# rkhosrowshahi/MO-VAE

Hardware: NVIDIA B200
Metric: aggregation_GBps (higher is better)
Workload: dtype f32

## Files before the change

mo-vae_b200/csrc/aggregate.cu:

```cuda
#include "recombine_device.cuh"
#include "solve_device.cuh"

namespace movae {

int fill_solve_params(int k, const movae_solve_spec* spec, SolveParams* out);
int check_solve_vectors(const SolveParams& p, const float* d_vec, const float* d_aux);

constexpr int kAggThreads = 256;
static_assert(kAggThreads == kGramThreads && kAggThreads == kRecThreads && kAggThreads == kSolveThreads, "one CTA shape");

struct AggArgs {
    const float* J;
    int64_t P, ldJ;
    unsigned char* ws;
    const float* vec;
    const float* aux;
    float* out;
    int accumulate;
    float* w_out;
    double* diag_out;
    double* G_out;
    int64_t window_gram;
    int64_t window_rec;
};

constexpr double kL2WindowFraction = 0.55;

struct PolicyIO {
    uint64_t pol;
    __device__ __forceinline__ float4 load(const float4* p) const { return ld_stream_f4(p, pol); }
    __device__ __forceinline__ float load(const float* p) const { return ld_stream_f1(p, pol); }
};

template <bool LAST_USE>
struct WindowSteps {
    int64_t window;
    __device__ __forceinline__ PolicyIO operator()(int64_t d) const {
        return {(d < window) == LAST_USE ? l2_policy_evict_first() : l2_policy_evict_normal()};
    }
};

template <int K>
__device__ __forceinline__ void aggregate_solve_phase(const SolveParams& sp, const P2PArgs& px, const float* vec, const float* aux,
                                                      float* w_out, double* diag_out, double* G_out, const GramWorkspace& ws,
                                                      unsigned int ready0, unsigned long long t_start) {
    __shared__ SolveSmem S;
    __shared__ double Gs[K * K];
    __shared__ unsigned long long seq_s;
    __shared__ int failed_s;
    const int tid = threadIdx.x;
    const unsigned long long t_in = global_timer_ns();
    gram_combine_partials<K>(ws.partials, Gs);
    if (tid == 0) { *ws.ticket = 0u; failed_s = 0; ws.stamps[4] = global_timer_ns(); }
    if (px.world > 0) {
        XchgBuffer* own = px.peers[px.rank];
        if (tid == 0) seq_s = own->step + 1;
        __syncthreads();
        const unsigned long long seq = seq_s;
        const int par = (int)(seq & 1ull);
        if (tid < K * K) {
            const double v = Gs[tid];
            for (int r = 0; r < px.world; ++r) st_relaxed_sys_f64(&px.peers[r]->slots[par][px.rank][tid], v);
        }
        __threadfence_system();
        __syncthreads();
        if (tid < px.world) st_release_sys_u64(&px.peers[tid]->flags[par][px.rank], seq);
        if (tid == 0) own->step = seq;
        if (tid < px.world && !wait_flag_sys(&own->flags[par][tid], seq, kExchangeTimeoutNs)) failed_s = 1;
        __syncthreads();
        if (tid < K * K) {
            double g = 0.0;
            for (int r = 0; r < px.world; ++r) g += ld_relaxed_sys_f64(&own->slots[par][r][tid]);
            Gs[tid] = g;
        }
        __syncthreads();
    }
    if (tid == 0) ws.stamps[5] = global_timer_ns();
    if (tid < MK * MK) {
        const int i = tid / MK, j = tid % MK;
        S.G[i][j] = (i < K && j < K) ? Gs[i * K + j] : 0.0;
    }
    if (G_out && tid < K * K) G_out[tid] = Gs[tid];
    __syncthreads();
    solve_block<K>(sp, S, vec, aux, failed_s != 0, tid);
    if (tid < K) {
        w_out[tid] = S.w[tid];
        if (sp.comfort) w_out[K + tid] = S.w2[tid];
    }
    __syncthreads();
    if (tid == 0) {
        ws.stamps[0] = t_start;
        ws.stamps[1] = t_in;
        ws.stamps[2] = global_timer_ns();
        __threadfence();
        st_release_gpu_u32(ws.ready, ready0 + 1u);
    }
    solve_diagnostics(sp, S, tid);
    __syncthreads();
    if (tid < MOVAE_DIAG_DOUBLES && diag_out) diag_out[tid] = S.dg[tid];
}

__device__ __forceinline__ void aggregate_prologue(const GramWorkspace& ws, unsigned int& ready0, unsigned long long& t_start) {
    if (threadIdx.x == 0) {
        ready0 = ld_acquire_gpu_u32(ws.ready);
        t_start = global_timer_ns();
    }
}

__device__ __forceinline__ void aggregate_wait_ready(const unsigned int* ready, unsigned int ready0) {
    if (threadIdx.x == 0) {
        const unsigned long long t0 = global_timer_ns();
        while (ld_acquire_gpu_u32(ready) == ready0) {
            __nanosleep(40);
            if (global_timer_ns() - t0 > 2ull * kExchangeTimeoutNs) break;
        }
    }
    __syncthreads();
}

__device__ __forceinline__ void aggregate_epilogue(const GramWorkspace& ws) {
    __syncthreads();
    if (threadIdx.x == 0) {
        if (atomicAdd(ws.exit, 1u) == gridDim.x - 1) {
            ws.stamps[3] = global_timer_ns();
            *ws.exit = 0u;
        }
    }
}

template <int K, int U1, int U2, bool VEC, int MINB>
__global__ void __launch_bounds__(kAggThreads, MINB)
aggregate_kernel(AggArgs a, SolveParams sp, P2PArgs px) {
    constexpr int NACC = GramAcc<K>::N;
    const GramWorkspace ws(a.ws);
    __shared__ unsigned int ready0;
    __shared__ unsigned long long t_start;
    __shared__ double red[kGramThreads / 32][NACC];
    __shared__ int is_last;
    aggregate_prologue(ws, ready0, t_start);

    double acc64[NACC];
#pragma unroll
    for (int i = 0; i < NACC; ++i) acc64[i] = 0.0;
    gram_stream_tiles<K, U1, VEC>(a.J, a.P, a.ldJ, acc64, WindowSteps<false>{a.window_gram});
    const bool last = gram_cta_partial_and_ticket<K>(acc64, ws.partials, ws.ticket, red, &is_last);

    if (last) aggregate_solve_phase<K>(sp, px, a.vec, a.aux, a.w_out, a.diag_out, a.G_out, ws, ready0, t_start);
    if (a.out == nullptr) return;

    recombine_tiles<K, U2, VEC>(
        a.J, a.P, a.ldJ, a.w_out, a.out, a.accumulate, [&] { if (!last) aggregate_wait_ready(ws.ready, ready0); },
        WindowSteps<true>{a.window_rec});
    aggregate_epilogue(ws);
}

template <int K, int U1, int U2, bool VEC, int MINB>
static int launch_aggregate(const AggArgs& a, const SolveParams& sp, const P2PArgs& px, cudaStream_t st) {
    constexpr auto kern = aggregate_kernel<K, U1, U2, VEC, MINB>;
    constexpr int W = VEC ? 4 : 1;
    static thread_local int l2_dev = -1, l2_bytes = 0;
    int dev = 0;
    MOVAE_CUDA_TRY(cudaGetDevice(&dev));
    if (l2_dev != dev) {
        MOVAE_CUDA_TRY(cudaDeviceGetAttribute(&l2_bytes, cudaDevAttrL2CacheSize, dev));
        l2_dev = dev;
    }
    const int64_t tile_items = (int64_t)kAggThreads * (U1 > U2 ? U1 : U2);
    unsigned int grid = 0;
    const int rc = persistent_grid<kern>(kAggThreads, (a.P / W + tile_items - 1) / tile_items, kGramMaxBlocks, &grid);
    if (rc != MOVAE_OK) return rc;
    AggArgs a_ = a;
    if (a.out != nullptr) {
        const double window = kL2WindowFraction * (double)l2_bytes / (double)grid;
        a_.window_gram = (int64_t)(window / (double)((int64_t)K * kAggThreads * U1 * W * sizeof(float)));
        a_.window_rec = (int64_t)(window / (double)((int64_t)K * kAggThreads * U2 * W * sizeof(float)));
    } else {
        a_.window_gram = a_.window_rec = INT64_MAX;
    }
    SolveParams sp_ = sp;
    P2PArgs px_ = px;
    void* params[] = {&a_, &sp_, &px_};
    MOVAE_CUDA_TRY(cudaLaunchCooperativeKernel(reinterpret_cast<const void*>(kern), dim3(grid), dim3(kAggThreads), params, 0, st));
    return MOVAE_OK;
}

struct SegArgs {
    movae_jac_segments segs;
    unsigned char* ws;
    const float* vec;
    const float* aux;
    float* out;
    int accumulate;
    float* w_out;
    double* diag_out;
    double* G_out;
};

struct SegRows {
    const float* const* rows;
    __device__ __forceinline__ const float* row(int i) const { return rows[i]; }
};

template <int K, int U, int MINB>
__global__ void __launch_bounds__(kAggThreads, MINB)
aggregate_seg_kernel(const __grid_constant__ SegArgs a, SolveParams sp, P2PArgs px) {
    constexpr int NACC = GramAcc<K>::N;
    constexpr int kTile = kAggThreads * U;
    const int tid = threadIdx.x;
    const GramWorkspace ws(a.ws);
    const int n_seg = a.segs.n_segments;

    __shared__ unsigned int ready0;
    __shared__ unsigned long long t_start;
    __shared__ double red[kGramThreads / 32][NACC];
    __shared__ int is_last;
    __shared__ int tile_start[MOVAE_MAX_SEGMENTS + 1];
    aggregate_prologue(ws, ready0, t_start);
    if (tid == 0) {
        int acc = 0;
        for (int s = 0; s < n_seg; ++s) {
            tile_start[s] = acc;
            acc += (int)(((a.segs.n[s] >> 2) + kTile - 1) / kTile);
        }
        tile_start[n_seg] = acc;
    }
    __syncthreads();
    const int n_tiles = tile_start[n_seg];
    auto segment_of = [&](int v) { int s = 0; while (v >= tile_start[s + 1]) ++s; return s; };

    double acc64[NACC];
#pragma unroll
    for (int i = 0; i < NACC; ++i) acc64[i] = 0.0;
    for (int v = blockIdx.x; v < n_tiles; v += gridDim.x) {
        const int s = segment_of(v);
        float acc[NACC];
#pragma unroll
        for (int q = 0; q < NACC; ++q) acc[q] = 0.f;
        gram_tile<K, U, true>(SegRows{a.segs.rows[s]}, (int64_t)(v - tile_start[s]) * kTile, a.segs.n[s] >> 2, false, acc);
#pragma unroll
        for (int q = 0; q < NACC; ++q) acc64[q] += (double)acc[q];
    }
    if (blockIdx.x == 0 && tid < 4 * n_seg) {
        const int s = tid >> 2;
        const int64_t c = (a.segs.n[s] & ~(int64_t)3) + (tid & 3);
        if (c < a.segs.n[s]) gram_column<K>(SegRows{a.segs.rows[s]}, c, acc64);
    }
    const bool last = gram_cta_partial_and_ticket<K>(acc64, ws.partials, ws.ticket, red, &is_last);

    if (last) aggregate_solve_phase<K>(sp, px, a.vec, a.aux, a.w_out, a.diag_out, a.G_out, ws, ready0, t_start);
    if (a.out == nullptr) return;

    auto wait = [&] { if (!last) aggregate_wait_ready(ws.ready, ready0); };
    float w[K];
    bool have_w = false;
    for (int v = n_tiles - 1 - (int)blockIdx.x; v >= 0; v -= gridDim.x) {
        const int s = segment_of(v);
        const int64_t t0 = (int64_t)(v - tile_start[s]) * kTile, n_items = a.segs.n[s] >> 2;
        RecTile<K, U, true> r;
        rec_load_tile<K, U, true>(r, SegRows{a.segs.rows[s]}, t0 + tid, t0, n_items, false);
        if (!have_w) {
            rec_read_weights<K>(a.w_out, wait, w);
            have_w = true;
        }
        rec_store_tile<K, U, true>(r, w, a.out + a.segs.out_off[s], t0 + tid, t0, n_items, false, a.accumulate);
    }
    if (!have_w) rec_read_weights<K>(a.w_out, wait, w);
    if (blockIdx.x == 0 && tid < 4 * n_seg) {
        const int s = tid >> 2;
        const int64_t c = (a.segs.n[s] & ~(int64_t)3) + (tid & 3);
        if (c < a.segs.n[s]) rec_column<K>(SegRows{a.segs.rows[s]}, w, a.out + a.segs.out_off[s], c, a.accumulate);
    }
    aggregate_epilogue(ws);
}

template <int K, int U, int MINB>
static int launch_aggregate_seg(const SegArgs& a, const SolveParams& sp, const P2PArgs& px, cudaStream_t st) {
    constexpr auto kern = aggregate_seg_kernel<K, U, MINB>;
    int64_t n_tiles = 0;
    for (int s = 0; s < a.segs.n_segments; ++s) n_tiles += ((a.segs.n[s] >> 2) + kAggThreads * U - 1) / (kAggThreads * U);
    unsigned int grid = 0;
    const int rc = persistent_grid<kern>(kAggThreads, n_tiles, kGramMaxBlocks, &grid);
    if (rc != MOVAE_OK) return rc;
    SegArgs a_ = a;
    SolveParams sp_ = sp;
    P2PArgs px_ = px;
    void* params[] = {&a_, &sp_, &px_};
    MOVAE_CUDA_TRY(cudaLaunchCooperativeKernel(reinterpret_cast<const void*>(kern), dim3(grid), dim3(kAggThreads), params, 0, st));
    return MOVAE_OK;
}

template <class CheckArgs>
static int check_fused_launch(const char* who, int k, const movae_solve_spec* spec, const float* d_vec, const float* d_aux,
                              CheckArgs check_args, const void* d_ws, size_t ws_bytes, const movae_p2p_ctx* ctx, SolveParams* sp,
                              P2PArgs* px) {
    int rc = fill_solve_params(k, spec, sp);
    if (rc == MOVAE_OK) rc = check_solve_vectors(*sp, d_vec, d_aux);
    if (rc == MOVAE_OK) rc = check_args();
    if (rc != MOVAE_OK) return rc;
    MOVAE_REQUIRE(d_ws != nullptr && ws_bytes >= movae_gram_workspace_bytes(k), MOVAE_ERR_WORKSPACE,
                  "%s: workspace too small (%zu < %zu)", who, ws_bytes, movae_gram_workspace_bytes(k));
    MOVAE_REQUIRE(reinterpret_cast<uintptr_t>(d_ws) % 8 == 0, MOVAE_ERR_WORKSPACE, "%s: workspace must be 8-byte aligned", who);
    *px = p2p_disabled();
    return ctx != nullptr ? make_p2p_args(ctx, px) : MOVAE_OK;
}

}

extern "C" {

int movae_aggregate_f32(const float* d_J, int k, int64_t P, int64_t ldJ, const movae_solve_spec* spec, const float* d_vec,
                        const float* d_aux, float* d_grad, int accumulate, float* d_w, double* d_diag, double* d_G, void* d_ws,
                        size_t ws_bytes, const movae_p2p_ctx* ctx, void* stream) {
    using namespace movae;
    SolveParams sp;
    P2PArgs px;
    const int rc = check_fused_launch("aggregate", k, spec, d_vec, d_aux, [&] {
        MOVAE_REQUIRE(P >= 0 && ldJ >= P, MOVAE_ERR_INVALID, "aggregate: need 0 <= P <= ldJ (P=%lld ldJ=%lld)", (long long)P, (long long)ldJ);
        MOVAE_REQUIRE(d_w != nullptr && (d_J != nullptr || P == 0), MOVAE_ERR_INVALID, "aggregate: null pointer");
        return MOVAE_OK;
    }, d_ws, ws_bytes, ctx, &sp, &px);
    if (rc != MOVAE_OK) return rc;
    AggArgs a;
    a.J = d_J;
    a.P = P;
    a.ldJ = ldJ;
    a.ws = static_cast<unsigned char*>(d_ws);
    a.vec = d_vec;
    a.aux = d_aux;
    a.out = d_grad;
    a.accumulate = accumulate;
    a.w_out = d_w;
    a.diag_out = d_diag;
    a.G_out = d_G;
    cudaStream_t st = static_cast<cudaStream_t>(stream);
    const bool vec = (reinterpret_cast<uintptr_t>(d_J) % 16 == 0) && (d_grad == nullptr || reinterpret_cast<uintptr_t>(d_grad) % 16 == 0) &&
                     (ldJ % 4 == 0 || k == 1);
    return dispatch_k(k, [&](auto kc) {
        constexpr int K = decltype(kc)::value;
        if (vec) {
            if constexpr (K <= 2) return launch_aggregate<K, 8, 4, true, 2>(a, sp, px, st);
            else if constexpr (K == 3) return launch_aggregate<K, 4, 4, true, 2>(a, sp, px, st);
            else if constexpr (K == 4) return launch_aggregate<K, 4, 2, true, 2>(a, sp, px, st);
            else return launch_aggregate<K, 2, 2, true, 1>(a, sp, px, st);
        } else {
            if constexpr (K <= 4) return launch_aggregate<K, 8, 8, false, 2>(a, sp, px, st);
            else return launch_aggregate<K, 4, 4, false, 1>(a, sp, px, st);
        }
    });
}

int movae_aggregate_segments_f32(const movae_jac_segments* segs, const movae_solve_spec* spec, const float* d_vec,
                                 const float* d_aux, float* d_grad, int accumulate, float* d_w, double* d_diag, double* d_G,
                                 void* d_ws, size_t ws_bytes, const movae_p2p_ctx* ctx, void* stream) {
    using namespace movae;
    MOVAE_REQUIRE(segs != nullptr, MOVAE_ERR_INVALID, "aggregate_segments: null segment table");
    const int k = segs->k;
    SolveParams sp;
    P2PArgs px;
    const int rc = check_fused_launch("aggregate_segments", k, spec, d_vec, d_aux, [&] {
        MOVAE_REQUIRE(segs->n_segments >= 1 && segs->n_segments <= MOVAE_MAX_SEGMENTS, MOVAE_ERR_UNSUPPORTED,
                      "aggregate_segments: %d segments outside 1..%d", segs->n_segments, MOVAE_MAX_SEGMENTS);
        MOVAE_REQUIRE(d_w != nullptr, MOVAE_ERR_INVALID, "aggregate_segments: null pointer");
        MOVAE_REQUIRE(d_grad == nullptr || reinterpret_cast<uintptr_t>(d_grad) % 16 == 0, MOVAE_ERR_INVALID,
                      "aggregate_segments: the gradient buffer must be 16-byte aligned");
        for (int s = 0; s < segs->n_segments; ++s) {
            MOVAE_REQUIRE(segs->n[s] >= 0 && segs->out_off[s] >= 0 && segs->out_off[s] % 4 == 0, MOVAE_ERR_INVALID,
                          "aggregate_segments: segment %d needs n >= 0 and an output offset that is a multiple of 4", s);
            for (int i = 0; i < k; ++i)
                MOVAE_REQUIRE(segs->rows[s][i] != nullptr && reinterpret_cast<uintptr_t>(segs->rows[s][i]) % 16 == 0, MOVAE_ERR_INVALID,
                              "aggregate_segments: row %d of segment %d must be a 16-byte aligned device pointer", i, s);
        }
        return MOVAE_OK;
    }, d_ws, ws_bytes, ctx, &sp, &px);
    if (rc != MOVAE_OK) return rc;
    SegArgs a;
    a.segs = *segs;
    a.ws = static_cast<unsigned char*>(d_ws);
    a.vec = d_vec;
    a.aux = d_aux;
    a.out = d_grad;
    a.accumulate = accumulate;
    a.w_out = d_w;
    a.diag_out = d_diag;
    a.G_out = d_G;
    cudaStream_t st = static_cast<cudaStream_t>(stream);
    return dispatch_k(k, [&](auto kc) {
        constexpr int K = decltype(kc)::value;
        if constexpr (K <= 3) return launch_aggregate_seg<K, 4, 2>(a, sp, px, st);
        else if constexpr (K == 4) return launch_aggregate_seg<K, 2, 2>(a, sp, px, st);
        else return launch_aggregate_seg<K, 2, 1>(a, sp, px, st);
    });
}

int movae_aggregate_timestamps(const void* d_ws, uint64_t h_stamps[6], void* stream) {
    using namespace movae;
    MOVAE_REQUIRE(d_ws != nullptr && h_stamps != nullptr, MOVAE_ERR_INVALID, "aggregate_timestamps: null pointer");
    cudaStream_t st = static_cast<cudaStream_t>(stream);
    MOVAE_CUDA_TRY(cudaMemcpyAsync(h_stamps, static_cast<const unsigned char*>(d_ws) + GramWorkspace::kStamps, 6 * sizeof(uint64_t),
                                   cudaMemcpyDeviceToHost, st));
    MOVAE_CUDA_TRY(cudaStreamSynchronize(st));
    return MOVAE_OK;
}

}
```

mo-vae_b200/csrc/common.cuh:

```cuda
#pragma once
#include <cuda_runtime.h>
#include <stdint.h>
#include <stdio.h>
#include <string.h>

#include <type_traits>

#include "../../include/movae_b200.h"

namespace movae {

void set_error(const char* fmt, ...);
int fail_cuda(cudaError_t e, const char* what);
int sm_count();

#define MOVAE_CUDA_TRY(expr)                                        \
    do {                                                            \
        cudaError_t _e = (expr);                                    \
        if (_e != cudaSuccess) return ::movae::fail_cuda(_e, #expr); \
    } while (0)

#define MOVAE_REQUIRE(cond, code, ...)          \
    do {                                        \
        if (!(cond)) {                          \
            ::movae::set_error(__VA_ARGS__);    \
            return (code);                      \
        }                                       \
    } while (0)

template <auto kern>
int persistent_grid(int threads, int64_t n_tiles, int64_t cap, unsigned int* grid) {
    static thread_local int occ_dev = -1, occ = 0;
    int dev = 0;
    MOVAE_CUDA_TRY(cudaGetDevice(&dev));
    if (occ_dev != dev) {
        MOVAE_CUDA_TRY(cudaOccupancyMaxActiveBlocksPerMultiprocessor(&occ, kern, threads, 0));
        if (occ < 1) occ = 1;
        occ_dev = dev;
    }
    const int sms = sm_count();
    MOVAE_REQUIRE(sms > 0, MOVAE_ERR_CUDA, "CUDA device query failed (no GPU?)");
    int64_t g = (int64_t)sms * occ;
    if (g > n_tiles) g = n_tiles;
    if (g > cap) g = cap;
    *grid = g > 1 ? (unsigned int)g : 1u;
    return MOVAE_OK;
}

template <int K = 1, class F>
int dispatch_k(int k, F&& f) {
    if constexpr (K == MOVAE_MAX_K) return f(std::integral_constant<int, K>{});
    else return k == K ? f(std::integral_constant<int, K>{}) : dispatch_k<K + 1>(k, f);
}

__device__ __forceinline__ float4 ld_stream_f4(const float4* p) {
    float4 v;
    asm volatile("ld.global.nc.L1::no_allocate.v4.f32 {%0,%1,%2,%3}, [%4];"
                 : "=f"(v.x), "=f"(v.y), "=f"(v.z), "=f"(v.w)
                 : "l"(p));
    return v;
}
__device__ __forceinline__ float ld_stream_f1(const float* p) {
    float v;
    asm volatile("ld.global.nc.L1::no_allocate.f32 %0, [%1];" : "=f"(v) : "l"(p));
    return v;
}
__device__ __forceinline__ uint64_t l2_policy_evict_first() {
    uint64_t p;
    asm("createpolicy.fractional.L2::evict_first.b64 %0, 1.0;" : "=l"(p));
    return p;
}
__device__ __forceinline__ uint64_t l2_policy_evict_normal() {
    uint64_t p;
    asm("createpolicy.fractional.L2::evict_normal.b64 %0, 1.0;" : "=l"(p));
    return p;
}
__device__ __forceinline__ float4 ld_stream_f4(const float4* p, uint64_t pol) {
    float4 v;
    asm volatile("ld.global.nc.L1::no_allocate.L2::cache_hint.v4.f32 {%0,%1,%2,%3}, [%4], %5;"
                 : "=f"(v.x), "=f"(v.y), "=f"(v.z), "=f"(v.w)
                 : "l"(p), "l"(pol));
    return v;
}
__device__ __forceinline__ float ld_stream_f1(const float* p, uint64_t pol) {
    float v;
    asm volatile("ld.global.nc.L1::no_allocate.L2::cache_hint.f32 %0, [%1], %2;" : "=f"(v) : "l"(p), "l"(pol));
    return v;
}
__device__ __forceinline__ void st_stream_f4(float4* p, float4 v) {
    asm volatile("st.global.cs.v4.f32 [%0], {%1,%2,%3,%4};" ::"l"(p), "f"(v.x), "f"(v.y), "f"(v.z), "f"(v.w)
                 : "memory");
}

struct XchgBuffer {
    double slots[2][MOVAE_MAX_WORLD][MOVAE_MAX_K * MOVAE_MAX_K];
    unsigned long long flags[2][MOVAE_MAX_WORLD];
    unsigned long long bar_flags[MOVAE_MAX_WORLD];
    unsigned long long step;
    unsigned long long bar_epoch;
};
struct P2PArgs {
    int rank, world;
    XchgBuffer* peers[MOVAE_MAX_WORLD];
};
__host__ __device__ inline P2PArgs p2p_disabled() {
    P2PArgs a;
    a.rank = 0;
    a.world = 0;
    for (int i = 0; i < MOVAE_MAX_WORLD; ++i) a.peers[i] = nullptr;
    return a;
}
int make_p2p_args(const movae_p2p_ctx* ctx, P2PArgs* out);

__device__ __forceinline__ void st_release_sys_u64(unsigned long long* p, unsigned long long v) {
    asm volatile("st.release.sys.global.u64 [%0], %1;" ::"l"(p), "l"(v) : "memory");
}
__device__ __forceinline__ unsigned long long ld_acquire_sys_u64(const unsigned long long* p) {
    unsigned long long v;
    asm volatile("ld.acquire.sys.global.u64 %0, [%1];" : "=l"(v) : "l"(p) : "memory");
    return v;
}
__device__ __forceinline__ double ld_relaxed_sys_f64(const double* p) {
    double v;
    asm volatile("ld.relaxed.sys.global.f64 %0, [%1];" : "=d"(v) : "l"(p) : "memory");
    return v;
}

__device__ __forceinline__ void st_relaxed_sys_f64(double* p, double v) {
    asm volatile("st.relaxed.sys.global.f64 [%0], %1;" ::"l"(p), "d"(v) : "memory");
}
__device__ __forceinline__ void st_release_gpu_u32(unsigned int* p, unsigned int v) {
    asm volatile("st.release.gpu.global.u32 [%0], %1;" ::"l"(p), "r"(v) : "memory");
}
__device__ __forceinline__ unsigned int ld_acquire_gpu_u32(const unsigned int* p) {
    unsigned int v;
    asm volatile("ld.acquire.gpu.global.u32 %0, [%1];" : "=r"(v) : "l"(p) : "memory");
    return v;
}
__device__ __forceinline__ unsigned long long global_timer_ns() {
    unsigned long long t;
    asm volatile("mov.u64 %0, %%globaltimer;" : "=l"(t));
    return t;
}
__device__ __forceinline__ bool wait_flag_sys(const unsigned long long* flag, unsigned long long want,
                                              unsigned long long timeout_ns) {
    if (ld_acquire_sys_u64(flag) >= want) return true;
    const unsigned long long t0 = global_timer_ns();
    while (ld_acquire_sys_u64(flag) < want) {
        if (global_timer_ns() - t0 > timeout_ns) return false;
    }
    return true;
}
constexpr unsigned long long kExchangeTimeoutNs = 20ull * 1000ull * 1000ull * 1000ull;

__device__ __forceinline__ double warp_sum(double v) {
#pragma unroll
    for (int o = 16; o > 0; o >>= 1) v += __shfl_xor_sync(0xffffffffu, v, o);
    return v;
}

}
```

mo-vae_b200/csrc/gram_device.cuh:

```cuda
#pragma once
#include "common.cuh"

namespace movae {

constexpr int kGramThreads = 256;
constexpr int kGramMaxBlocks = 2048;
constexpr int kGramHeaderBytes = 256;
constexpr int kGramChain = 64;

struct GramWorkspace {
    static constexpr int kTicket = 0, kExit = 4, kReady = 128, kStamps = 192;
    unsigned int* ticket;
    unsigned int* exit;
    unsigned int* ready;
    unsigned long long* stamps;
    double* partials;
    __host__ __device__ explicit GramWorkspace(void* ws) {
        unsigned char* b = static_cast<unsigned char*>(ws);
        ticket = reinterpret_cast<unsigned int*>(b + kTicket);
        exit = reinterpret_cast<unsigned int*>(b + kExit);
        ready = reinterpret_cast<unsigned int*>(b + kReady);
        stamps = reinterpret_cast<unsigned long long*>(b + kStamps);
        partials = reinterpret_cast<double*>(b + kGramHeaderBytes);
    }
};
static_assert(GramWorkspace::kStamps + 6 * 8 <= kGramHeaderBytes, "the timestamps fit the header");

struct FlatRows {
    const float* J;
    int64_t ldJ;
    __device__ __forceinline__ const float* row(int i) const { return J + i * ldJ; }
};

template <int K>
struct GramAcc {
    static constexpr int N = K * (K + 1) / 2;
};

template <int K>
__device__ __forceinline__ void gram_fma(float (&acc)[GramAcc<K>::N], const float (&x)[K]) {
    int a = 0;
#pragma unroll
    for (int i = 0; i < K; ++i)
#pragma unroll
        for (int j = i; j < K; ++j) { acc[a] = fmaf(x[i], x[j], acc[a]); ++a; }
}

struct RRSchedule {
    int64_t rounds;
    int64_t rem_lo, rem_hi;
};
__device__ __forceinline__ RRSchedule rr_schedule(int64_t n_items, int64_t tile_items, int64_t b, int64_t g) {
    RRSchedule s;
    s.rounds = (n_items / tile_items) / g;
    const int64_t r0 = s.rounds * g * tile_items;
    const int64_t m = (((n_items - r0) + g - 1) / g + 7) & ~(int64_t)7;
    s.rem_lo = r0 + b * m < n_items ? r0 + b * m : n_items;
    s.rem_hi = s.rem_lo + m < n_items ? s.rem_lo + m : n_items;
    return s;
}

struct PlainTileIO {
    __device__ __forceinline__ float4 load(const float4* p) const { return ld_stream_f4(p); }
    __device__ __forceinline__ float load(const float* p) const { return ld_stream_f1(p); }
};
struct PlainSteps {
    __device__ __forceinline__ PlainTileIO operator()(int64_t) const { return {}; }
};

template <int K, int U, bool VEC, class Rows, class IO = PlainTileIO>
__device__ __forceinline__ void gram_tile(const Rows& rows, int64_t t0, int64_t hi, bool full, float (&acc)[GramAcc<K>::N],
                                          IO io = {}) {
    const int64_t base = t0 + threadIdx.x;
    if constexpr (VEC) {
        float4 v[K][U];
        if (full) {
#pragma unroll
            for (int i = 0; i < K; ++i)
#pragma unroll
                for (int u = 0; u < U; ++u)
                    v[i][u] = io.load(reinterpret_cast<const float4*>(rows.row(i)) + base + u * kGramThreads);
        } else {
#pragma unroll
            for (int i = 0; i < K; ++i)
#pragma unroll
                for (int u = 0; u < U; ++u) {
                    const int64_t idx = base + u * kGramThreads;
                    v[i][u] = idx < hi ? io.load(reinterpret_cast<const float4*>(rows.row(i)) + idx) : make_float4(0.f, 0.f, 0.f, 0.f);
                }
        }
#pragma unroll
        for (int u = 0; u < U; ++u) {
            float x[K];
#pragma unroll
            for (int i = 0; i < K; ++i) x[i] = v[i][u].x;
            gram_fma<K>(acc, x);
#pragma unroll
            for (int i = 0; i < K; ++i) x[i] = v[i][u].y;
            gram_fma<K>(acc, x);
#pragma unroll
            for (int i = 0; i < K; ++i) x[i] = v[i][u].z;
            gram_fma<K>(acc, x);
#pragma unroll
            for (int i = 0; i < K; ++i) x[i] = v[i][u].w;
            gram_fma<K>(acc, x);
        }
    } else {
        float v[K][U];
#pragma unroll
        for (int i = 0; i < K; ++i)
#pragma unroll
            for (int u = 0; u < U; ++u) {
                const int64_t idx = base + u * kGramThreads;
                v[i][u] = idx < hi ? io.load(rows.row(i) + idx) : 0.f;
            }
#pragma unroll
        for (int u = 0; u < U; ++u) {
            float x[K];
#pragma unroll
            for (int i = 0; i < K; ++i) x[i] = v[i][u];
            gram_fma<K>(acc, x);
        }
    }
}

template <int K, class Rows>
__device__ __forceinline__ void gram_column(const Rows& rows, int64_t c, double (&acc64)[GramAcc<K>::N]) {
    constexpr int NACC = GramAcc<K>::N;
    float x[K];
    float acc[NACC];
#pragma unroll
    for (int a = 0; a < NACC; ++a) acc[a] = 0.f;
#pragma unroll
    for (int i = 0; i < K; ++i) x[i] = rows.row(i)[c];
    gram_fma<K>(acc, x);
#pragma unroll
    for (int a = 0; a < NACC; ++a) acc64[a] += (double)acc[a];
}

template <int K, int U, bool VEC, class Steps = PlainSteps>
__device__ __forceinline__ void gram_stream_tiles(const float* __restrict__ J, int64_t P, int64_t ldJ,
                                                  double (&acc64)[GramAcc<K>::N], Steps steps = {}) {
    constexpr int NACC = GramAcc<K>::N;
    constexpr int W = VEC ? 4 : 1;
    constexpr int FLUSH = kGramChain / (W * U) > 0 ? kGramChain / (W * U) : 1;
    const int tid = threadIdx.x;
    const int64_t n_items = P / W;
    constexpr int64_t tile_items = (int64_t)kGramThreads * U;
    const RRSchedule sch = rr_schedule(n_items, tile_items, blockIdx.x, gridDim.x);
    const int64_t n_steps = sch.rounds + (sch.rem_hi > sch.rem_lo ? 1 : 0);
    const FlatRows rows{J, ldJ};

    int64_t r = 0;
    while (r < sch.rounds) {
        float acc[NACC];
#pragma unroll
        for (int a = 0; a < NACC; ++a) acc[a] = 0.f;
#pragma unroll 1
        for (int f = 0; f < FLUSH && r < sch.rounds; ++f, ++r) {
            const int64_t t0 = (r * gridDim.x + blockIdx.x) * tile_items;
            gram_tile<K, U, VEC>(rows, t0, t0 + tile_items, true, acc, steps(n_steps - 1 - r));
        }
#pragma unroll
        for (int a = 0; a < NACC; ++a) acc64[a] += (double)acc[a];
    }
    if (sch.rem_hi > sch.rem_lo) {
        float acc[NACC];
#pragma unroll
        for (int a = 0; a < NACC; ++a) acc[a] = 0.f;
        gram_tile<K, U, VEC>(rows, sch.rem_lo, sch.rem_hi, false, acc, steps(0));
#pragma unroll
        for (int a = 0; a < NACC; ++a) acc64[a] += (double)acc[a];
    }

    if (VEC && blockIdx.x == 0 && tid < (int)(P - n_items * W)) gram_column<K>(rows, n_items * W + tid, acc64);
}

template <int K>
__device__ __forceinline__ bool gram_cta_partial_and_ticket(const double (&acc64)[GramAcc<K>::N], double* __restrict__ partials,
                                                            unsigned int* __restrict__ counter,
                                                            double (*red)[GramAcc<K>::N], int* is_last_smem) {
    constexpr int NACC = GramAcc<K>::N;
    const int tid = threadIdx.x, warp = tid >> 5, lane = tid & 31;
#pragma unroll
    for (int a = 0; a < NACC; ++a) {
        const double s = warp_sum(acc64[a]);
        if (lane == 0) red[warp][a] = s;
    }
    __syncthreads();
    if (tid < NACC) {
        double s = 0.0;
#pragma unroll
        for (int w = 0; w < kGramThreads / 32; ++w) s += red[w][tid];
        partials[(int64_t)blockIdx.x * NACC + tid] = s;
    }
    __threadfence();
    __syncthreads();
    if (tid == 0) *is_last_smem = (atomicAdd(counter, 1u) == gridDim.x - 1);
    __syncthreads();
    return *is_last_smem != 0;
}

template <int K>
__device__ __forceinline__ void gram_combine_partials(const double* __restrict__ partials, double* __restrict__ Gs) {
    constexpr int NACC = GramAcc<K>::N;
    const int tid = threadIdx.x, warp = tid >> 5, lane = tid & 31;
    __threadfence();
    for (int a = warp; a < NACC; a += kGramThreads / 32) {
        double s0 = 0.0, s1 = 0.0, s2 = 0.0, s3 = 0.0;
        const int g = (int)gridDim.x;
        for (int b = lane; b < g; b += 128) {
            const double v0 = __ldcg(&partials[(int64_t)b * NACC + a]);
            const double v1 = b + 32 < g ? __ldcg(&partials[(int64_t)(b + 32) * NACC + a]) : 0.0;
            const double v2 = b + 64 < g ? __ldcg(&partials[(int64_t)(b + 64) * NACC + a]) : 0.0;
            const double v3 = b + 96 < g ? __ldcg(&partials[(int64_t)(b + 96) * NACC + a]) : 0.0;
            s0 += v0; s1 += v1; s2 += v2; s3 += v3;
        }
        double s = (s0 + s1) + (s2 + s3);
        s = warp_sum(s);
        if (lane == 0) {
            int i = 0, rem = a;
            while (rem >= K - i) { rem -= K - i; ++i; }
            const int j = i + rem;
            Gs[i * K + j] = s;
            Gs[j * K + i] = s;
        }
    }
    __syncthreads();
}

}
```

mo-vae_b200/csrc/recombine_device.cuh:

```cuda
#pragma once
#include <type_traits>

#include "gram_device.cuh"

namespace movae {

constexpr int kRecThreads = 256;

template <int K, int U, bool VEC>
struct RecTile {
    using T = typename std::conditional<VEC, float4, float>::type;
    T v[K][U];
};

template <int K, int U, bool VEC, class Rows, class IO = PlainTileIO>
__device__ __forceinline__ void rec_load_tile(RecTile<K, U, VEC>& r, const Rows& rows, int64_t base, int64_t lo, int64_t hi,
                                              bool full, IO io = {}) {
#pragma unroll
    for (int i = 0; i < K; ++i)
#pragma unroll
        for (int u = 0; u < U; ++u) {
            const int64_t idx = base + u * kRecThreads;
            if constexpr (VEC)
                r.v[i][u] = (full || (idx >= lo && idx < hi)) ? io.load(reinterpret_cast<const float4*>(rows.row(i)) + idx)
                                                    : make_float4(0.f, 0.f, 0.f, 0.f);
            else
                r.v[i][u] = (full || (idx >= lo && idx < hi)) ? io.load(rows.row(i) + idx) : 0.f;
        }
}

template <int K, int U, bool VEC>
__device__ __forceinline__ void rec_store_tile(const RecTile<K, U, VEC>& r, const float (&w)[K], float* __restrict__ out,
                                               int64_t base, int64_t lo, int64_t hi, bool full, int accumulate) {
#pragma unroll
    for (int u = 0; u < U; ++u) {
        const int64_t idx = base + u * kRecThreads;
        if (!full && (idx < lo || idx >= hi)) continue;
        if constexpr (VEC) {
            float4 o;
            o.x = w[0] * r.v[0][u].x; o.y = w[0] * r.v[0][u].y; o.z = w[0] * r.v[0][u].z; o.w = w[0] * r.v[0][u].w;
#pragma unroll
            for (int i = 1; i < K; ++i) {
                o.x = fmaf(w[i], r.v[i][u].x, o.x); o.y = fmaf(w[i], r.v[i][u].y, o.y);
                o.z = fmaf(w[i], r.v[i][u].z, o.z); o.w = fmaf(w[i], r.v[i][u].w, o.w);
            }
            float4* dst = reinterpret_cast<float4*>(out) + idx;
            if (accumulate) {
                const float4 old = *dst;
                o.x += old.x; o.y += old.y; o.z += old.z; o.w += old.w;
            }
            st_stream_f4(dst, o);
        } else {
            float o = w[0] * r.v[0][u];
#pragma unroll
            for (int i = 1; i < K; ++i) o = fmaf(w[i], r.v[i][u], o);
            if (accumulate) o += out[idx];
            out[idx] = o;
        }
    }
}

template <int K, class Rows>
__device__ __forceinline__ void rec_column(const Rows& rows, const float (&w)[K], float* __restrict__ out, int64_t c,
                                           int accumulate) {
    float o = w[0] * rows.row(0)[c];
#pragma unroll
    for (int q = 1; q < K; ++q) o = fmaf(w[q], rows.row(q)[c], o);
    if (accumulate) o += out[c];
    out[c] = o;
}

template <int K, class Ready>
__device__ __forceinline__ void rec_read_weights(const float* w_dev, Ready ready, float (&w)[K]) {
    ready();
#pragma unroll
    for (int q = 0; q < K; ++q) w[q] = __ldcg(w_dev + q);
}

template <int K, int U, bool VEC, class Ready, class Steps = PlainSteps>
__device__ __forceinline__ void recombine_tiles(const float* __restrict__ J, int64_t P, int64_t ldJ, const float* w_dev,
                                                float* __restrict__ out, int accumulate, Ready ready, Steps steps = {}) {
    constexpr int W = VEC ? 4 : 1;
    const int tid = threadIdx.x;
    const int64_t n_items = P / W;
    constexpr int64_t tile_items = (int64_t)kRecThreads * U;
    const RRSchedule sch = rr_schedule(n_items, tile_items, blockIdx.x, gridDim.x);
    const bool has_rem = sch.rem_hi > sch.rem_lo;
    const FlatRows rows{J, ldJ};
    const int64_t n_steps = sch.rounds + (has_rem ? 1 : 0);
    auto t0_of = [&](int64_t i) -> int64_t {
        if (has_rem) { if (i == 0) return sch.rem_lo; --i; }
        return ((sch.rounds - 1 - i) * gridDim.x + blockIdx.x) * tile_items;
    };
    auto hi_of = [&](int64_t i, int64_t t0) -> int64_t { return (has_rem && i == 0) ? sch.rem_hi : t0 + tile_items; };
    auto full_of = [&](int64_t i) -> bool { return !(has_rem && i == 0); };

    RecTile<K, U, VEC> ra, rb;
    int64_t i = 0;
    int64_t ta = 0, tb = 0;
    if (n_steps > 0) { ta = t0_of(0); rec_load_tile<K, U, VEC>(ra, rows, ta + tid, ta, hi_of(0, ta), full_of(0), steps(0)); }
    float w[K];
    rec_read_weights<K>(w_dev, ready, w);
    while (i < n_steps) {
        const bool has_b = i + 1 < n_steps;
        if (has_b) { tb = t0_of(i + 1); rec_load_tile<K, U, VEC>(rb, rows, tb + tid, tb, hi_of(i + 1, tb), full_of(i + 1), steps(i + 1)); }
        rec_store_tile<K, U, VEC>(ra, w, out, ta + tid, ta, hi_of(i, ta), full_of(i), accumulate);
        if (!has_b) break;
        if (i + 2 < n_steps) { ta = t0_of(i + 2); rec_load_tile<K, U, VEC>(ra, rows, ta + tid, ta, hi_of(i + 2, ta), full_of(i + 2), steps(i + 2)); }
        rec_store_tile<K, U, VEC>(rb, w, out, tb + tid, tb, hi_of(i + 1, tb), full_of(i + 1), accumulate);
        i += 2;
    }
    if (VEC && blockIdx.x == 0 && tid < (int)(P - n_items * W)) rec_column<K>(rows, w, out, n_items * W + tid, accumulate);
}

}
```

Measured before the change: 7006.

## Prefetch recombine tiles into L2 during solve wait and enable PDL launch

While non-last CTAs spin waiting for the solve, they now detect that the solve phase started and issue bulk L2 prefetches for recombine tiles just beyond the L2-resident window. The evict-first window is extended by the prefetch span. The kernel is also launched with programmatic stream serialization via griddepcontrol so the next launch can overlap this kernel's tail. This adds a solving counter to the workspace. It risks L2 thrash if the prefetch span plus window exceeds capacity, and PDL could interact oddly with cooperative launch.

```diff
diff --git a/mo-vae_b200/csrc/aggregate.cu b/mo-vae_b200/csrc/aggregate.cu
--- a/mo-vae_b200/csrc/aggregate.cu
+++ b/mo-vae_b200/csrc/aggregate.cu
@@ -22,9 +22,11 @@
     double* G_out;
     int64_t window_gram;
     int64_t window_rec;
+    int64_t prefetch_rec;
 };
 
 constexpr double kL2WindowFraction = 0.55;
+constexpr double kL2PrefetchFraction = 0.2;
 
 struct PolicyIO {
     uint64_t pol;
@@ -50,6 +52,7 @@
     __shared__ int failed_s;
     const int tid = threadIdx.x;
     const unsigned long long t_in = global_timer_ns();
+    if (tid == 0) atomicAdd(ws.solving, 1u);
     gram_combine_partials<K>(ws.partials, Gs);
     if (tid == 0) { *ws.ticket = 0u; failed_s = 0; ws.stamps[4] = global_timer_ns(); }
     if (px.world > 0) {
@@ -107,10 +110,21 @@
     }
 }
 
-__device__ __forceinline__ void aggregate_wait_ready(const unsigned int* ready, unsigned int ready0) {
+struct NoSolveHook {
+    __device__ __forceinline__ void operator()() const {}
+};
+
+template <class OnSolve = NoSolveHook>
+__device__ __forceinline__ void aggregate_wait_ready(const GramWorkspace& ws, unsigned int ready0, unsigned int solving0 = 0,
+                                                     OnSolve on_solve = {}) {
     if (threadIdx.x == 0) {
         const unsigned long long t0 = global_timer_ns();
-        while (ld_acquire_gpu_u32(ready) == ready0) {
+        bool hooked = std::is_same<OnSolve, NoSolveHook>::value;
+        while (ld_acquire_gpu_u32(ws.ready) == ready0) {
+            if (!hooked && *reinterpret_cast<volatile unsigned int*>(ws.solving) != solving0) {
+                on_solve();
+                hooked = true;
+            }
             __nanosleep(40);
             if (global_timer_ns() - t0 > 2ull * kExchangeTimeoutNs) break;
         }
@@ -131,6 +145,7 @@
 template <int K, int U1, int U2, bool VEC, int MINB>
 __global__ void __launch_bounds__(kAggThreads, MINB)
 aggregate_kernel(AggArgs a, SolveParams sp, P2PArgs px) {
+    grid_dependency_wait();
     constexpr int NACC = GramAcc<K>::N;
     const GramWorkspace ws(a.ws);
     __shared__ unsigned int ready0;
@@ -138,6 +153,8 @@
     __shared__ double red[kGramThreads / 32][NACC];
     __shared__ int is_last;
     aggregate_prologue(ws, ready0, t_start);
+    unsigned int solving0 = 0;
+    if (threadIdx.x == 0) solving0 = *reinterpret_cast<volatile unsigned int*>(ws.solving);
 
     double acc64[NACC];
 #pragma unroll
@@ -149,8 +166,16 @@
     if (a.out == nullptr) return;
 
     recombine_tiles<K, U2, VEC>(
-        a.J, a.P, a.ldJ, a.w_out, a.out, a.accumulate, [&] { if (!last) aggregate_wait_ready(ws.ready, ready0); },
-        WindowSteps<true>{a.window_rec});
+        a.J, a.P, a.ldJ, a.w_out, a.out, a.accumulate,
+        [&] {
+            if (!last) {
+                aggregate_wait_ready(ws, ready0, solving0, [&] {
+                    if constexpr (VEC) rec_prefetch_l2<K, U2>(a.J, a.P, a.ldJ, a.window_rec, a.window_rec + a.prefetch_rec);
+                });
+            }
+            grid_launch_dependents();
+        },
+        WindowSteps<true>{a.window_rec + a.prefetch_rec});
     aggregate_epilogue(ws);
 }
 
@@ -171,16 +196,28 @@
     if (rc != MOVAE_OK) return rc;
     AggArgs a_ = a;
     if (a.out != nullptr) {
-        const double window = kL2WindowFraction * (double)l2_bytes / (double)grid;
-        a_.window_gram = (int64_t)(window / (double)((int64_t)K * kAggThreads * U1 * W * sizeof(float)));
-        a_.window_rec = (int64_t)(window / (double)((int64_t)K * kAggThreads * U2 * W * sizeof(float)));
+        const double per_cta = (double)l2_bytes / (double)grid;
+        const double rec_step = (double)((int64_t)K * kAggThreads * U2 * W * sizeof(float));
+        a_.window_gram = (int64_t)(kL2WindowFraction * per_cta / (double)((int64_t)K * kAggThreads * U1 * W * sizeof(float)));
+        a_.window_rec = (int64_t)(kL2WindowFraction * per_cta / rec_step);
+        a_.prefetch_rec = VEC ? (int64_t)(kL2PrefetchFraction * per_cta / rec_step) : 0;
     } else {
         a_.window_gram = a_.window_rec = INT64_MAX;
-    }
-    SolveParams sp_ = sp;
-    P2PArgs px_ = px;
-    void* params[] = {&a_, &sp_, &px_};
-    MOVAE_CUDA_TRY(cudaLaunchCooperativeKernel(reinterpret_cast<const void*>(kern), dim3(grid), dim3(kAggThreads), params, 0, st));
+        a_.prefetch_rec = 0;
+    }
+    cudaLaunchAttribute attrs[2];
+    attrs[0].id = cudaLaunchAttributeCooperative;
+    attrs[0].val.cooperative = 1;
+    attrs[1].id = cudaLaunchAttributeProgrammaticStreamSerialization;
+    attrs[1].val.programmaticStreamSerializationAllowed = 1;
+    cudaLaunchConfig_t cfg = {};
+    cfg.gridDim = dim3(grid);
+    cfg.blockDim = dim3(kAggThreads);
+    cfg.dynamicSmemBytes = 0;
+    cfg.stream = st;
+    cfg.attrs = attrs;
+    cfg.numAttrs = 2;
+    MOVAE_CUDA_TRY(cudaLaunchKernelEx(&cfg, kern, a_, sp, px));
     return MOVAE_OK;
 }
 
@@ -250,7 +287,7 @@
     if (last) aggregate_solve_phase<K>(sp, px, a.vec, a.aux, a.w_out, a.diag_out, a.G_out, ws, ready0, t_start);
     if (a.out == nullptr) return;
 
-    auto wait = [&] { if (!last) aggregate_wait_ready(ws.ready, ready0); };
+    auto wait = [&] { if (!last) aggregate_wait_ready(ws, ready0); };
     float w[K];
     bool have_w = false;
     for (int v = n_tiles - 1 - (int)blockIdx.x; v >= 0; v -= gridDim.x) {
diff --git a/mo-vae_b200/csrc/common.cuh b/mo-vae_b200/csrc/common.cuh
--- a/mo-vae_b200/csrc/common.cuh
+++ b/mo-vae_b200/csrc/common.cuh
@@ -87,6 +87,11 @@
     asm volatile("ld.global.nc.L1::no_allocate.L2::cache_hint.f32 %0, [%1], %2;" : "=f"(v) : "l"(p), "l"(pol));
     return v;
 }
+__device__ __forceinline__ void prefetch_l2_bulk(const void* p, uint32_t bytes, uint64_t pol) {
+    asm volatile("cp.async.bulk.prefetch.L2.global.L2::cache_hint [%0], %1, %2;" ::"l"(p), "r"(bytes), "l"(pol) : "memory");
+}
+__device__ __forceinline__ void grid_dependency_wait() { asm volatile("griddepcontrol.wait;" ::: "memory"); }
+__device__ __forceinline__ void grid_launch_dependents() { asm volatile("griddepcontrol.launch_dependents;" ::: "memory"); }
 __device__ __forceinline__ void st_stream_f4(float4* p, float4 v) {
     asm volatile("st.global.cs.v4.f32 [%0], {%1,%2,%3,%4};" ::"l"(p), "f"(v.x), "f"(v.y), "f"(v.z), "f"(v.w)
                  : "memory");
diff --git a/mo-vae_b200/csrc/gram_device.cuh b/mo-vae_b200/csrc/gram_device.cuh
--- a/mo-vae_b200/csrc/gram_device.cuh
+++ b/mo-vae_b200/csrc/gram_device.cuh
@@ -9,10 +9,11 @@
 constexpr int kGramChain = 64;
 
 struct GramWorkspace {
-    static constexpr int kTicket = 0, kExit = 4, kReady = 128, kStamps = 192;
+    static constexpr int kTicket = 0, kExit = 4, kReady = 128, kSolving = 132, kStamps = 192;
     unsigned int* ticket;
     unsigned int* exit;
     unsigned int* ready;
+    unsigned int* solving;
     unsigned long long* stamps;
     double* partials;
     __host__ __device__ explicit GramWorkspace(void* ws) {
@@ -20,6 +21,7 @@
         ticket = reinterpret_cast<unsigned int*>(b + kTicket);
         exit = reinterpret_cast<unsigned int*>(b + kExit);
         ready = reinterpret_cast<unsigned int*>(b + kReady);
+        solving = reinterpret_cast<unsigned int*>(b + kSolving);
         stamps = reinterpret_cast<unsigned long long*>(b + kStamps);
         partials = reinterpret_cast<double*>(b + kGramHeaderBytes);
     }
diff --git a/mo-vae_b200/csrc/recombine_device.cuh b/mo-vae_b200/csrc/recombine_device.cuh
--- a/mo-vae_b200/csrc/recombine_device.cuh
+++ b/mo-vae_b200/csrc/recombine_device.cuh
@@ -77,40 +77,62 @@
     for (int q = 0; q < K; ++q) w[q] = __ldcg(w_dev + q);
 }
 
+struct RecDeal {
+    RRSchedule sch;
+    int64_t tile_items, n_steps;
+    bool has_rem;
+    __device__ __forceinline__ RecDeal(int64_t n_items, int64_t tile_items_) : tile_items(tile_items_) {
+        sch = rr_schedule(n_items, tile_items, blockIdx.x, gridDim.x);
+        has_rem = sch.rem_hi > sch.rem_lo;
+        n_steps = sch.rounds + (has_rem ? 1 : 0);
+    }
+    __device__ __forceinline__ int64_t t0(int64_t i) const {
+        if (has_rem) { if (i == 0) return sch.rem_lo; --i; }
+        return ((sch.rounds - 1 - i) * gridDim.x + blockIdx.x) * tile_items;
+    }
+    __device__ __forceinline__ bool full(int64_t i) const { return !(has_rem && i == 0); }
+    __device__ __forceinline__ int64_t hi(int64_t i, int64_t t0) const { return full(i) ? t0 + tile_items : sch.rem_hi; }
+};
+
 template <int K, int U, bool VEC, class Ready, class Steps = PlainSteps>
 __device__ __forceinline__ void recombine_tiles(const float* __restrict__ J, int64_t P, int64_t ldJ, const float* w_dev,
                                                 float* __restrict__ out, int accumulate, Ready ready, Steps steps = {}) {
     constexpr int W = VEC ? 4 : 1;
     const int tid = threadIdx.x;
     const int64_t n_items = P / W;
-    constexpr int64_t tile_items = (int64_t)kRecThreads * U;
-    const RRSchedule sch = rr_schedule(n_items, tile_items, blockIdx.x, gridDim.x);
-    const bool has_rem = sch.rem_hi > sch.rem_lo;
+    const RecDeal deal(n_items, (int64_t)kRecThreads * U);
     const FlatRows rows{J, ldJ};
-    const int64_t n_steps = sch.rounds + (has_rem ? 1 : 0);
-    auto t0_of = [&](int64_t i) -> int64_t {
-        if (has_rem) { if (i == 0) return sch.rem_lo; --i; }
-        return ((sch.rounds - 1 - i) * gridDim.x + blockIdx.x) * tile_items;
-    };
-    auto hi_of = [&](int64_t i, int64_t t0) -> int64_t { return (has_rem && i == 0) ? sch.rem_hi : t0 + tile_items; };
-    auto full_of = [&](int64_t i) -> bool { return !(has_rem && i == 0); };
+    const int64_t n_steps = deal.n_steps;
 
     RecTile<K, U, VEC> ra, rb;
     int64_t i = 0;
     int64_t ta = 0, tb = 0;
-    if (n_steps > 0) { ta = t0_of(0); rec_load_tile<K, U, VEC>(ra, rows, ta + tid, ta, hi_of(0, ta), full_of(0), steps(0)); }
+    if (n_steps > 0) { ta = deal.t0(0); rec_load_tile<K, U, VEC>(ra, rows, ta + tid, ta, deal.hi(0, ta), deal.full(0), steps(0)); }
     float w[K];
     rec_read_weights<K>(w_dev, ready, w);
     while (i < n_steps) {
         const bool has_b = i + 1 < n_steps;
-        if (has_b) { tb = t0_of(i + 1); rec_load_tile<K, U, VEC>(rb, rows, tb + tid, tb, hi_of(i + 1, tb), full_of(i + 1), steps(i + 1)); }
-        rec_store_tile<K, U, VEC>(ra, w, out, ta + tid, ta, hi_of(i, ta), full_of(i), accumulate);
+        if (has_b) { tb = deal.t0(i + 1); rec_load_tile<K, U, VEC>(rb, rows, tb + tid, tb, deal.hi(i + 1, tb), deal.full(i + 1), steps(i + 1)); }
+        rec_store_tile<K, U, VEC>(ra, w, out, ta + tid, ta, deal.hi(i, ta), deal.full(i), accumulate);
         if (!has_b) break;
-        if (i + 2 < n_steps) { ta = t0_of(i + 2); rec_load_tile<K, U, VEC>(ra, rows, ta + tid, ta, hi_of(i + 2, ta), full_of(i + 2), steps(i + 2)); }
-        rec_store_tile<K, U, VEC>(rb, w, out, tb + tid, tb, hi_of(i + 1, tb), full_of(i + 1), accumulate);
+        if (i + 2 < n_steps) { ta = deal.t0(i + 2); rec_load_tile<K, U, VEC>(ra, rows, ta + tid, ta, deal.hi(i + 2, ta), deal.full(i + 2), steps(i + 2)); }
+        rec_store_tile<K, U, VEC>(rb, w, out, tb + tid, tb, deal.hi(i + 1, tb), deal.full(i + 1), accumulate);
         i += 2;
     }
     if (VEC && blockIdx.x == 0 && tid < (int)(P - n_items * W)) rec_column<K>(rows, w, out, n_items * W + tid, accumulate);
 }
 
+template <int K, int U>
+__device__ __forceinline__ void rec_prefetch_l2(const float* J, int64_t P, int64_t ldJ, int64_t first, int64_t last) {
+    const RecDeal deal(P / 4, (int64_t)kRecThreads * U);
+    if (last > deal.n_steps) last = deal.n_steps;
+    const uint64_t pol = l2_policy_evict_normal();
+    for (int64_t s = first; s < last; ++s) {
+        const int64_t t0 = deal.t0(s);
+        const uint32_t bytes = (uint32_t)((deal.hi(s, t0) - t0) * (int64_t)sizeof(float4));
+#pragma unroll
+        for (int i = 0; i < K; ++i) prefetch_l2_bulk(reinterpret_cast<const float4*>(J + i * ldJ) + t0, bytes, pol);
+    }
 }
+
+}
```

After: 7002, median of 6. About the same (-0.1%).
